# thenoobychocobo/gpt2-image-captioning

Measured on AMD Instinct MI355X. Metric: training images/sec + greedy captions/sec, GPT2-small+CLIP-B/32 at 1/2/4/8 GPU, higher is better.
Workload: dtype bf16

## Files before the change

### gpt2-image-captioning_amd/csrc/elementwise.hip

```cpp
#include "common.h"

#include <math.h>

namespace icap {

static inline hipStream_t S_(void* s) { return reinterpret_cast<hipStream_t>(s); }
static inline unsigned nblk(int64_t n, int per, int cap = 65535) {
  int64_t b = (n + per - 1) / per;
  if (b < 1) b = 1;
  if (b > cap) b = cap;
  return (unsigned)b;
}

__device__ __forceinline__ float block_sum256(float v, float* red) {
  v = wave_sum(v);
  const int lane = threadIdx.x & 63, w = threadIdx.x >> 6;
  __syncthreads();
  if (lane == 0) red[w] = v;
  __syncthreads();
  float r = red[0] + red[1] + red[2] + red[3];
  return r;
}

template <typename T>
__global__ void gpt2_embed_kernel(int B, int P, int L, int D, const T* __restrict__ prefix, int64_t pbs,
                                  const T* __restrict__ wte, const T* __restrict__ wpe,
                                  const int64_t* __restrict__ ids, T* __restrict__ x, uint32_t thr,
                                  float inv_keep, uint64_t seed0, const uint64_t* seed_ptr, uint64_t offset,
                                  const int32_t* __restrict__ seq_off, const int32_t* __restrict__ seq_len) {
  const int S = P + L, D4 = D >> 2;
  const uint64_t seed = thr ? eff_seed(seed0, seed_ptr) : 0ull;
  const int64_t total = (int64_t)B * S * D4;
  for (int64_t i = (int64_t)blockIdx.x * blockDim.x + threadIdx.x; i < total; i += (int64_t)gridDim.x * blockDim.x) {
    const int64_t prow = i / D4;
    const int c = (int)(i - prow * D4) * 4;
    const int b = (int)(prow / S), t = (int)(prow - (int64_t)b * S);
    int64_t row = prow;
    if (seq_off) {
      if (t >= seq_len[b]) continue;
      row = (int64_t)seq_off[b] + t;
    }
    float v[4], w[4];
    if (t < P) io<T>::ld4(prefix + (int64_t)b * pbs + (int64_t)t * D + c, v);
    else io<T>::ld4(wte + ids[(int64_t)b * L + (t - P)] * D + c, v);
    io<T>::ld4(wpe + (int64_t)t * D + c, w);
#pragma unroll
    for (int e = 0; e < 4; ++e) {
      v[e] += w[e];
      if (thr) v[e] *= drop_scale(seed, offset + (uint64_t)(row * D + c + e), thr, inv_keep);
    }
    io<T>::st4(x + row * D + c, v);
  }
}

template <typename T>
// ... 495 lines not shown
  const double lr = (double)lr0 * lam;
  const double t = (double)(k + 1);
  const double bc1 = 1.0 - pow((double)beta1, t);
  const double bc2 = 1.0 - pow((double)beta2, t);
  st->norm = norm;
  st->clip = clip;
  st->lr = (float)lr;
  st->step_size = (float)(lr / bc1);
  st->bc2_sqrt = (float)sqrt(bc2);
  st->decay = (float)(1.0 - lr * (double)wd);
  st->step = k + 1;
}

__device__ __forceinline__ void adam_one(float& p, float g, float& m, float& v, float clip, float decay, float w1,
                                         float b2, float w2, float step_size, float bc2s, float eps) {
  g *= clip;
  p *= decay;
  m = m + w1 * (g - m);
  v = v * b2 + w2 * (g * g);
  const float denom = sqrtf(v) / bc2s + eps;
  p = p + (-step_size) * (m / denom);
}

__global__ __launch_bounds__(256) void adam_update_kernel(int64_t n, float* __restrict__ P, const float* __restrict__ G,
                                                         float* __restrict__ M1, float* __restrict__ M2,
                                                         bf16_t* __restrict__ out16, const AdamState* __restrict__ st,
                                                         float beta1, float beta2, float eps) {
  const float clip = st->clip, decay = st->decay, step_size = st->step_size, bc2s = st->bc2_sqrt;
  const float w1 = 1.f - beta1, w2 = 1.f - beta2;
  const int64_t n4 = n >> 2;
  for (int64_t i = (int64_t)blockIdx.x * 256 + threadIdx.x; i < n4; i += (int64_t)gridDim.x * 256) {
    float4 p = reinterpret_cast<float4*>(P)[i];
    const float4 g = reinterpret_cast<const float4*>(G)[i];
    float4 m = reinterpret_cast<float4*>(M1)[i];
    float4 v = reinterpret_cast<float4*>(M2)[i];
    adam_one(p.x, g.x, m.x, v.x, clip, decay, w1, beta2, w2, step_size, bc2s, eps);
    adam_one(p.y, g.y, m.y, v.y, clip, decay, w1, beta2, w2, step_size, bc2s, eps);
    adam_one(p.z, g.z, m.z, v.z, clip, decay, w1, beta2, w2, step_size, bc2s, eps);
    adam_one(p.w, g.w, m.w, v.w, clip, decay, w1, beta2, w2, step_size, bc2s, eps);
    reinterpret_cast<float4*>(P)[i] = p;
    reinterpret_cast<float4*>(M1)[i] = m;
    reinterpret_cast<float4*>(M2)[i] = v;
    if (out16) {
      const float o[4] = {p.x, p.y, p.z, p.w};
      io<bf16_t>::st4(out16 + 4 * i, o);
    }
  }
  if (blockIdx.x == 0) {
    for (int64_t i = 4 * n4 + threadIdx.x; i < n; i += 256) {
      float p = P[i], m = M1[i], v = M2[i];
      adam_one(p, G[i], m, v, clip, decay, w1, beta2, w2, step_size, bc2s, eps);
      P[i] = p; M1[i] = m; M2[i] = v;
      if (out16) out16[i] = f2bf(p);
    }
  }
}

template <typename T>
__global__ __launch_bounds__(256) void transpose_kernel(int64_t rows, int64_t cols, const T* __restrict__ src,
                                                       int64_t lds, T* __restrict__ dst, int64_t ldd,
                                                       int64_t rows_pad) {
  __shared__ T tile[64][65];
  const int64_t r0 = (int64_t)blockIdx.y * 64, c0 = (int64_t)blockIdx.x * 64;
  const int tx = threadIdx.x & 63, ty = threadIdx.x >> 6;
  for (int i = ty; i < 64; i += 4) {
    const int64_t r = r0 + i, c = c0 + tx;
    T v = (T)0;
    if (r < rows && c < cols) v = src[r * lds + c];
    tile[i][tx] = v;
  }
  __syncthreads();
  for (int i = ty; i < 64; i += 4) {
    const int64_t c = c0 + i, r = r0 + tx;
    if (c < cols && r < rows_pad) dst[c * ldd + r] = tile[tx][i];
  }
}

template <typename T>
__global__ __launch_bounds__(256) void colsum_kernel(int64_t M, int64_t N, const T* __restrict__ src, int64_t ld,
                                                    int64_t rows_per_chunk, float* __restrict__ partial) {
  __shared__ float red[4][64];
  const int tx = threadIdx.x & 63, ty = threadIdx.x >> 6;
  const int64_t c = (int64_t)blockIdx.x * 64 + tx;
  const int64_t m0 = (int64_t)blockIdx.y * rows_per_chunk;
  int64_t m1 = m0 + rows_per_chunk;
  if (m1 > M) m1 = M;
  float a = 0.f;
  if (c < N)
    for (int64_t m = m0 + ty; m < m1; m += 4) a += io<T>::ld(src + m * ld + c);
  red[ty][tx] = a;
  __syncthreads();
  if (ty == 0 && c < N) partial[(int64_t)blockIdx.y * N + c] = red[0][tx] + red[1][tx] + red[2][tx] + red[3][tx];
}

constexpr int T16_TLD = 68;
__device__ __forceinline__ void transpose16_tile(int64_t rows, int64_t cols, const uint16_t* __restrict__ src,
                                                 int64_t lds, uint16_t* __restrict__ dst, int64_t ldd, int64_t r0,
                                                 int64_t c0, uint16_t* tile) {
  constexpr int TLD = T16_TLD;
#pragma unroll
  for (int h = 0; h < 2; ++h) {
    const int idx = threadIdx.x + 256 * h;
    const int r = idx >> 3, ch = idx & 7;
    uint4 v = make_uint4(0, 0, 0, 0);
    if (r0 + r < rows && c0 + 8 * ch < cols) v = *reinterpret_cast<const uint4*>(src + (r0 + r) * lds + c0 + 8 * ch);
    uint2* t = reinterpret_cast<uint2*>(&tile[r * TLD + 8 * ch]);
// ... 745 lines not shown
  ICAP_REQUIRE(V > 0 && ld >= V && ld % 4 == 0, "icap_cross_entropy: ld must be >= V and a multiple of 4");
  if (rows <= 0) return ICAP_OK;
  ICAP_REQUIRE(rows < (1ll << 31), "icap_cross_entropy: too many rows");
  float* lrows = reinterpret_cast<float*>(workspace);
  const bool reg = dtype == ICAP_BF16 && V <= 8 * 512 * 13 && ld % 8 == 0 &&
                   (reinterpret_cast<uintptr_t>(logits) & 15) == 0 &&
                   (dlogits == nullptr || (reinterpret_cast<uintptr_t>(dlogits) & 15) == 0);
  if (reg) {
    hipLaunchKernelGGL(ce_bf16_reg_kernel<13>, dim3((unsigned)rows), dim3(512), 0, S_(stream), V,
                       reinterpret_cast<const bf16_t*>(logits), ld, labels, n_valid, lrows,
                       reinterpret_cast<bf16_t*>(dlogits), grad_scale, rows_dev);
  } else {
    DISPATCH_T(dtype, hipLaunchKernelGGL(ce_kernel<T>, dim3((unsigned)rows), dim3(256), 0, S_(stream), V, CTP(logits),
                                         ld, labels, n_valid, lrows, TP(dlogits), grad_scale, rows_dev));
  }
  int rc = check_launch("icap_cross_entropy");
  if (rc) return rc;
  hipLaunchKernelGGL(ce_reduce_kernel, dim3(1), dim3(256), 0, S_(stream), rows, lrows, n_valid, loss, rows_dev);
  return check_launch("icap_cross_entropy(reduce)");
}

extern "C" size_t icap_adamw_workspace_bytes(int64_t n) {
  (void)n;
  return SQ_BLOCKS * sizeof(float);
}

static int sq_partials(int64_t n, const float* x, float* partial, hipStream_t s, int* nparts) {
  const int nb = (int)nblk(n / 4 + 1, 256, SQ_BLOCKS);
  hipLaunchKernelGGL(sqnorm_partial_kernel, dim3(nb), dim3(256), 0, s, n, x, partial);
  *nparts = nb;
  return check_launch("sqnorm");
}

extern "C" int icap_sqnorm(int64_t n, const float* x, float* out, void* workspace, void* stream) {
  ICAP_REQUIRE(x && out && workspace, "icap_sqnorm: null pointer");
  ICAP_REQUIRE((reinterpret_cast<uintptr_t>(x) & 15) == 0, "icap_sqnorm: x must be 16-byte aligned");
  int np = 0;
  float* partial = reinterpret_cast<float*>(workspace);
  int rc = sq_partials(n, x, partial, S_(stream), &np);
  if (rc) return rc;
  hipLaunchKernelGGL(adam_finalize_kernel, dim3(1), dim3(256), 0, S_(stream), np, partial, (AdamState*)nullptr, out,
                     0.f, 0.f, 0.f, 0.f, 0.f, (int64_t)0, (int64_t)0);
  return check_launch("icap_sqnorm");
}

extern "C" int icap_adamw_step(const icap_adamw_args* a, void* workspace, void* stream) {
  ICAP_REQUIRE(a && workspace, "icap_adamw_step: null args/workspace");
  ICAP_REQUIRE(a->params && a->grads && a->exp_avg && a->exp_avg_sq && a->state, "icap_adamw_step: null pointer");
  ICAP_REQUIRE(((reinterpret_cast<uintptr_t>(a->params) | reinterpret_cast<uintptr_t>(a->grads) |
                 reinterpret_cast<uintptr_t>(a->exp_avg) | reinterpret_cast<uintptr_t>(a->exp_avg_sq)) & 15) == 0,
               "icap_adamw_step: buffers must be 16-byte aligned");
  ICAP_REQUIRE(a->bf16_out == nullptr || (reinterpret_cast<uintptr_t>(a->bf16_out) & 7) == 0,
               "icap_adamw_step: bf16_out must be 8-byte aligned");
  if (a->n <= 0) return ICAP_OK;
  hipStream_t s = S_(stream);
  float* partial = reinterpret_cast<float*>(workspace);
  int np = 0;
  int rc = sq_partials(a->n, a->grads, partial, s, &np);
  if (rc) return rc;
  hipLaunchKernelGGL(adam_finalize_kernel, dim3(1), dim3(256), 0, s, np, partial, (AdamState*)a->state,
                     (float*)nullptr, a->lr, a->beta1, a->beta2, a->weight_decay, a->max_norm, a->num_warmup_steps,
                     a->num_training_steps);
  rc = check_launch("icap_adamw_step(finalize)");
  if (rc) return rc;
  hipLaunchKernelGGL(adam_update_kernel, dim3(nblk(a->n / 4 + 1, 256, 4096)), dim3(256), 0, s, a->n, a->params,
                     a->grads, a->exp_avg, a->exp_avg_sq, (bf16_t*)a->bf16_out, (const AdamState*)a->state, a->beta1,
                     a->beta2, a->eps);
  return check_launch("icap_adamw_step(update)");
}

extern "C" int icap_transpose(int32_t dtype, int64_t rows, int64_t cols, const void* src, int64_t lds, void* dst,
                              int64_t ldd, int64_t rows_pad, void* stream) {
  ICAP_REQUIRE(src && dst && rows_pad >= rows, "icap_transpose: bad args");
  if (rows_pad == 0 || cols == 0) return ICAP_OK;
  dim3 grid((unsigned)((cols + 63) / 64), (unsigned)((rows_pad + 63) / 64));
  ICAP_REQUIRE(grid.y < 65536, "icap_transpose: too many rows");
  const bool vec = dtype == ICAP_BF16 && cols % 8 == 0 && lds % 8 == 0 && ldd % 8 == 0 && rows_pad % 64 == 0 &&
                   (reinterpret_cast<uintptr_t>(src) & 15) == 0 && (reinterpret_cast<uintptr_t>(dst) & 15) == 0;
  if (vec)
    hipLaunchKernelGGL(transpose16_vec_kernel, grid, dim3(256), 0, S_(stream), rows, cols, (const uint16_t*)src, lds,
                       (uint16_t*)dst, ldd);
  else if (dtype == ICAP_BF16)
    hipLaunchKernelGGL(transpose_kernel<uint16_t>, grid, dim3(256), 0, S_(stream), rows, cols, (const uint16_t*)src,
                       lds, (uint16_t*)dst, ldd, rows_pad);
  else
    hipLaunchKernelGGL(transpose_kernel<uint32_t>, grid, dim3(256), 0, S_(stream), rows, cols, (const uint32_t*)src,
                       lds, (uint32_t*)dst, ldd, rows_pad);
  return check_launch("icap_transpose");
}

extern "C" int icap_transpose_batch(int32_t n, const icap_transpose_item* items, void* stream) {
  ICAP_REQUIRE(n >= 0 && (n == 0 || items), "icap_transpose_batch: bad args");
  for (int32_t i0 = 0; i0 < n; i0 += T16_BATCH) {
    const int m = n - i0 < T16_BATCH ? n - i0 : T16_BATCH;
    Transpose16Batch b;
    b.n = 0;
    b.off[0] = 0;
    for (int j = 0; j < m; ++j) {
      const icap_transpose_item& it = items[i0 + j];
      ICAP_REQUIRE(it.src && it.dst && it.rows >= 0 && it.cols >= 0, "icap_transpose_batch: bad item");
      if (it.rows == 0 || it.cols == 0) continue;
      const bool vec = it.cols % 8 == 0 && it.lds % 8 == 0 && it.ldd % 8 == 0 && it.rows % 64 == 0 &&
                       it.lds >= it.cols && it.ldd >= it.rows && (reinterpret_cast<uintptr_t>(it.src) & 15) == 0 &&
                       (reinterpret_cast<uintptr_t>(it.dst) & 15) == 0;
      if (!vec) {
        const int rc = icap_transpose(ICAP_BF16, it.rows, it.cols, it.src, it.lds, it.dst, it.ldd, it.rows, stream);
        if (rc) return rc;
        continue;
      }
      const int k = b.n++;
      b.src[k] = static_cast<const uint16_t*>(it.src);
      b.dst[k] = static_cast<uint16_t*>(it.dst);
      b.rows[k] = it.rows; b.cols[k] = it.cols; b.lds[k] = it.lds; b.ldd[k] = it.ldd;
      b.off[k + 1] = b.off[k] + ((it.cols + 63) / 64) * (it.rows / 64);
    }
    if (b.n == 0) continue;
    ICAP_REQUIRE(b.off[b.n] < (1ll << 31), "icap_transpose_batch: too many tiles");
    hipLaunchKernelGGL(transpose16_batch_kernel, dim3((unsigned)b.off[b.n]), dim3(256), 0, S_(stream), b);
    const int rc = check_launch("icap_transpose_batch");
    if (rc) return rc;
  }
// ... 288 lines not shown
```

### gpt2-image-captioning_amd/icap/_lib.py

```python

from __future__ import annotations

import ctypes as C
import os

import torch

_HERE = os.path.dirname(os.path.abspath(__file__))
LIB_PATH = os.environ.get("ICAP_LIB") or os.path.join(_HERE, "libicap_hip.so")

F32, BF16, FP8_MX = 0, 1, 2
ACT_NONE, ACT_GELU_NEW, ACT_RELU, ACT_QUICK_GELU, ACT_TANH, ACT_GELU_ERF = 0, 1, 2, 3, 4, 5
AGG_MEAN, AGG_MAX, AGG_SUM_NORM = 0, 1, 2

vp = C.c_void_p
i32, i64, u64, f32, sz = C.c_int32, C.c_int64, C.c_uint64, C.c_float, C.c_size_t
pi32 = C.POINTER(C.c_int32)
pi64 = C.POINTER(C.c_int64)


class GemmArgs(C.Structure):
    _fields_ = [
        ("M", i64), ("N", i64), ("K", i64),
        ("in_dtype", i32), ("c_dtype", i32),
# ... 14 lines not shown
        ("trans_ab", i32),
        ("ln_gamma", vp), ("ln_beta", vp), ("ln_eps", f32),
        ("path", i32),
        ("a_scale", vp), ("b_scale", vp),
        ("m_hint", i64),
        ("tickets", vp), ("tickets_len", i64),
        ("ln_wsum", vp),
        ("ln_stats_out", vp), ("ln_stats_in", vp), ("ln_mean_out", vp), ("ln_rstd_out", vp),
        ("diag_stamps", vp),
    ]


class LnParamItem(C.Structure):
    _fields_ = [("workspace", vp), ("rows", i64), ("D", i64), ("dgamma", vp), ("dbeta", vp), ("overwrite", i32)]


class TransposeItem(C.Structure):
    _fields_ = [("src", vp), ("lds", i64), ("dst", vp), ("ldd", i64), ("rows", i64), ("cols", i64)]


class ColsumItem(C.Structure):
    _fields_ = [("src", vp), ("ld", i64), ("N", i64), ("out", vp)]


class AttnArgs(C.Structure):
    _fields_ = [
        ("dtype", i32),
        ("B", i32), ("S", i32), ("H", i32), ("hd", i32),
        ("row_stride_b", i64), ("row_stride_s", i64),
        ("qkv", vp), ("ld_qkv", i64),
        ("out", vp), ("ld_out", i64),
        ("lse", vp),
        ("key_mask", vp),
        ("causal", i32),
        ("scale", f32),
        ("drop_p", f32), ("seed", u64), ("offset", u64),
        ("seed_ptr", vp),
        ("dout", vp), ("ld_dout", i64),
        ("dqkv", vp), ("ld_dqkv", i64),
        ("seq_off", vp), ("seq_len", vp),
        ("short_only", i32),
    ]


class AdamWArgs(C.Structure):
    _fields_ = [
        ("n", i64),
        ("params", vp), ("grads", vp), ("exp_avg", vp), ("exp_avg_sq", vp),
        ("bf16_out", vp),
        ("state", vp),
        ("lr", f32), ("beta1", f32), ("beta2", f32), ("eps", f32), ("weight_decay", f32),
        ("max_norm", f32),
        ("num_warmup_steps", i64), ("num_training_steps", i64),
    ]


class BeamArgs(C.Structure):
    _fields_ = [
        ("B", i32), ("W", i32), ("V", i32), ("max_len", i32),
        ("eos", i32), ("length_penalty", f32),
        ("K", i32),
        ("T", i32),
        ("top_val", vp), ("top_idx", vp), ("top_m", vp), ("top_ls", vp),
        ("ws", vp),
        ("dtype", i32), ("D", i32), ("n_positions", i32),
        ("wte", vp), ("wpe", vp), ("x", vp),
    ]


SIGNATURES = {
    "icap_last_error": (C.c_char_p, []),
    "icap_version": (C.c_int, []),
    "icap_device_arch_ok": (C.c_int, []),
    "icap_gemm": (C.c_int, [C.POINTER(GemmArgs), vp]),
    "icap_gemm_group": (C.c_int, [C.POINTER(GemmArgs), C.c_int32, vp]),
    "icap_gemm_kernel_name": (C.c_char_p, [C.POINTER(GemmArgs)]),
    "icap_gemm_plan_info": (C.c_int, [C.POINTER(GemmArgs), vp, vp]),
    "icap_mx_scale_bytes": (sz, [i64, i64]),
    "icap_quantize_mx": (C.c_int, [i32, i64, i64, vp, i64, vp, i64, vp, vp, vp]),
    "icap_layernorm_fwd": (C.c_int, [i32, i64, i64, vp, i64, vp, vp, f32, vp, i64, vp, vp, vp, vp, vp]),
    "icap_layernorm_bwd_workspace_bytes": (sz, [i64, i64]),
    "icap_layernorm_bwd": (C.c_int, [i32, i64, i64, vp, i64, vp, vp, vp, vp, i64, vp, i64, vp, i64, vp,
                                     f32, u64, u64, vp, vp, vp, vp, vp, vp, i32, vp]),
    "icap_ln_param_reduce_batch": (C.c_int, [i32, C.POINTER(LnParamItem), vp]),
    "icap_attention_fwd": (C.c_int, [C.POINTER(AttnArgs), vp]),
    "icap_attention_bwd": (C.c_int, [C.POINTER(AttnArgs), vp]),
    "icap_attention_decode": (C.c_int, [i32, i32, i32, i32, i32, vp, i64, vp, i64, f32, vp]),
    "icap_attention_decode_anc": (C.c_int, [i32, i32, i32, i32, i32, vp, i64, vp, vp, i64, f32, vp]),
    "icap_beam_workspace_bytes": (C.c_size_t, [i32, i32, i32, i32]),
    "icap_beam_layout": (C.c_int, [i32, i32, i32, i32, vp]),
    "icap_beam_init": (C.c_int, [C.POINTER(BeamArgs), i32, vp]),
    "icap_beam_rowtop": (C.c_int, [i32, i64, i64, vp, i64, i32, vp, vp, vp, vp, vp]),
    "icap_beam_update": (C.c_int, [C.POINTER(BeamArgs), i32, i32, vp]),
    "icap_beam_finalize": (C.c_int, [C.POINTER(BeamArgs), vp, vp, vp]),
    "icap_gpt2_embed": (C.c_int, [i32, i32, i32, i32, i32, vp, i64, vp, vp, vp, vp, f32, u64, u64, vp, vp, vp, vp]),
    "icap_embedding_scatter_add": (C.c_int, [i32, i32, i32, i32, i32, vp, vp, vp, vp]),
    "icap_caption_prep": (C.c_int, [i32, i32, i32, vp, vp, vp, vp, vp, vp, vp, vp]),
    "icap_caption_pack": (C.c_int, [i32, i32, i32, vp, vp, vp, vp, vp, vp, vp, vp, vp, vp, vp]),
    "icap_rows_unpack": (C.c_int, [i32, i32, i32, i32, vp, vp, vp, vp, i64, vp]),
    "icap_cross_entropy_workspace_bytes": (sz, [i64]),
    "icap_cross_entropy": (C.c_int, [i32, i64, i64, vp, i64, vp, vp, vp, vp, f32, vp, vp, vp]),
    "icap_adamw_workspace_bytes": (sz, [i64]),
    "icap_adamw_step": (C.c_int, [C.POINTER(AdamWArgs), vp, vp]),
    "icap_sqnorm": (C.c_int, [i64, vp, vp, vp, vp]),
    "icap_transpose": (C.c_int, [i32, i64, i64, vp, i64, vp, i64, i64, vp]),
    "icap_transpose_batch": (C.c_int, [i32, vp, vp]),
    "icap_colsum_workspace_bytes": (sz, [i64, i64]),
# ... 76 lines not shown
```

### gpt2-image-captioning_amd/icap/engine.py

```python

from __future__ import annotations

from types import SimpleNamespace
from typing import List, Optional, Tuple

import torch

from . import ops
from .mapper import DWHelper, MLPMapperCore, TransformerMapperCore
from .models import _embedding_grads

SHORT_ONLY = True
GRAD_OVERWRITE = True

Tensor = torch.Tensor


def _async_src(t: Tensor) -> bool:
    return t.device.type != "cpu" or t.is_pinned()


class CaptionTrainer:
    def __init__(self, model, batch_size: int, caption_len: int, *, lr: float = 1e-4, weight_decay: float = 0.01,
                 betas=(0.9, 0.999), eps: float = 1e-8, max_norm: float = 1.0, num_warmup_steps: int = 0,
                 num_training_steps: int = 1, dropout: bool = True, seed: int = 0, clip_model=None,
                 grad_accum_steps: int = 1, process_group=None, compact_head: bool = True,
                 pack_rows: bool = True, dp_overlap: bool = True, dp_bf16: bool = False, force_overlap: bool = False,
                 mapper_dw: str = "fused"):
        self.model = model
        self.dtype = model.compute_dtype
        self.B, self.Lc = batch_size, caption_len
        self.hp = SimpleNamespace(lr=lr, weight_decay=weight_decay, betas=betas, eps=eps, max_norm=max_norm,
                                  num_warmup_steps=num_warmup_steps, num_training_steps=num_training_steps)
        self.dropout = dropout
        self.seed = seed
        self.grad_accum_steps = grad_accum_steps
        self.pg = process_group
        self.world = 1
        self.distributed = process_group is not None or (torch.distributed.is_available()
                                                         and torch.distributed.is_initialized())
        if self.distributed:
            self.world = torch.distributed.get_world_size(process_group)
            broadcast_replicas([model] + ([clip_model] if clip_model is not None else []), process_group)
        self.force_overlap = bool(force_overlap) and self.distributed
        self.dev = model.device
        flat = model.flat()
        self.flat = flat
        self.mcore = model.mapping_network.core(self.dtype, flat)
        self.clip = clip_model.core(self.dtype) if clip_model is not None else None
        self.gpt_trainable = not model.freeze_gpt_weights
        if self.gpt_trainable:
            model.gpt.invalidate_core()
            self.gcore = model.gpt.core(self.dtype)
            model.gpt.invalidate_core()
            self.gcore.bind_flat(flat)
            compact_head = False
        else:
            self.gcore = model.gpt.core(self.dtype)
        B, Lc = batch_size, caption_len
        P = model.total_prefix_length
        self.P = P
        per_layer = (dict(per_layer_grads=mapper_dw in ("side", "group")) if isinstance(self.mcore, TransformerMapperCore)
                     else {})
        self.mws = self.mcore.alloc(B, train=True, **per_layer)
        self.gws = self.gcore.alloc_train(B, P, Lc, keep_for_dw=self.gpt_trainable, compact_head=compact_head,
                                          pack=pack_rows)
# ... 118 lines not shown
                d_pre = st.d_emb.view(B, S * D)[:, : P * D]
                mc.backward_from(d_pre[:, : Pm * D], S * D, self.mws, self.emb_c, self.mgrads, self.dwh)

            segs.append((self._ranges_mapper[0], mlp))
        last_rng, last_fn = segs[-1]

        def last():
            last_fn()
            self.loss_sum.add_(self.gws.loss)

        segs[-1] = (last_rng, last)
        return segs

    def _overwrite_ok(self) -> bool:
        return GRAD_OVERWRITE and isinstance(self.mcore, TransformerMapperCore) and not self.gpt_trainable

    def _front(self, zero: bool, grad_scale: float):
        B, P, D = self.B, self.P, self.gcore.D
        model = self.model
        if zero and not self._overwrite_ok():
            self.flat.flat_grad.zero_()
        if self.clip is not None:
            emb = self.clip.run(self.cws, self.pixels)
            ops.convert(emb, self.emb_c)
        else:
            ops.convert(self.emb, self.emb_c)
        if self.dropout:
            ops.counter_increment(self.counter)
        mc, gc = self.mcore, self.gcore
        mc.forward(self.mws, self.emb_c, self.mdr, train=True)
        pre, pbs = mc.prefix_view(self.mws)
        if model.task_prefix_embeds is not None:
            Pm = mc.P
            ops.convert(_rows_view(pre, B, Pm * D, pbs), self.pre.view(B, P * D)[:, : Pm * D])
            ops.broadcast_rows(model.task_prefix_embeds.data, self.pre.view(-1)[Pm * D:], B, P * D)
            pre, pbs = self.pre, P * D
        gc.forward_train(self.gws, pre, pbs, self.ids, self.mask, self.labels, self.gdr, fuse_dlogits=True,
                         grad_scale=grad_scale)
        S = self.gws.S
        d_emb = gc.backward(self.gws, self.gdr, self.gws.key_mask, self.gws.logits, grads=self.ggrads,
                            dw=self.dwh if self.gpt_trainable else None)
        if self.gpt_trainable:
            _embedding_grads(d_emb, self.ids, B, P, self.Lc, D, self.ggrads, self.dwh)
        d_pre = d_emb.view(B, S * D)[:, : P * D]
        Pm = mc.P
        if model.task_prefix_embeds is not None:
            ops.colsum(d_emb.view(B, S * D)[:, Pm * D: P * D], self.task_grad.view(-1), self.dwh.cs_ws,
                       accumulate=not (zero and self._overwrite_ok()), M=B, N=(P - Pm) * D)
        if isinstance(mc, TransformerMapperCore):
            Hl, Sm = mc.Hl, mc.S
            ops.convert(d_pre[:, : Pm * D], self.mws.dout.view(B, Sm * D)[:, Hl * D:])
        return d_emb

    def _optimizer(self) -> None:
        hp, f = self.hp, self.flat
        ops.adamw_step(f.flat, f.flat_grad, f.exp_avg, f.exp_avg_sq, self.adam_state, self.adam_ws, lr=hp.lr,
                       betas=hp.betas, eps=hp.eps, weight_decay=hp.weight_decay, max_norm=hp.max_norm,
                       num_warmup_steps=hp.num_warmup_steps, num_training_steps=hp.num_training_steps,
                       bf16_out=f.flat_c)
        self.mcore.refresh_transposes()
        if self.gpt_trainable:
            self.gcore.refresh_from_flat()

    def _allreduce(self) -> None:
        if self.world > 1:
            if self.dp_bf16:
                g = self.flat.flat_grad
                self._to16(g, 0, g.numel())
                torch.distributed.all_reduce(self._g16, group=self.pg)
                self._from16(g, [(0, g.numel())])
            else:
                torch.distributed.all_reduce(self.flat.flat_grad, group=self.pg)

    def _to16(self, g, lo: int, hi: int) -> None:
        if self._g16 is None:
            self._g16 = torch.empty(g.numel(), dtype=torch.bfloat16, device=g.device)
        if g.is_cuda:
            ops.convert(g[lo:hi].view(1, -1), self._g16[lo:hi].view(1, -1))
        else:
            self._g16[lo:hi].copy_(g[lo:hi])

    def _from16(self, g, ranges) -> None:
        for lo, hi in ranges:
            if g.is_cuda:
                ops.convert(self._g16[lo:hi].view(1, -1), g[lo:hi].view(1, -1))
            else:
                g[lo:hi].copy_(self._g16[lo:hi])

    def _bucket(self, ranges, works) -> None:
        g = self.flat.flat_grad
        if not ranges:
            return
        src = (lambda lo, hi: self._g16[lo:hi]) if self.dp_bf16 else (lambda lo, hi: g[lo:hi])
        if g.is_cuda:
            if self._comm is None:
                self._comm = torch.cuda.Stream(g.device)
            ev = torch.cuda.Event()
            ev.record()
            with torch.cuda.stream(self._comm):
                self._comm.wait_event(ev)
                for lo, hi in ranges:
                    if self.dp_bf16:
                        self._to16(g, lo, hi)
                    works.append(torch.distributed.all_reduce(src(lo, hi), group=self.pg, async_op=True))
        else:
            for lo, hi in ranges:
                if self.dp_bf16:
                    self._to16(g, lo, hi)
                works.append(torch.distributed.all_reduce(src(lo, hi), group=self.pg, async_op=True))
        if self.dp_bf16:
            self._pending16.extend(ranges)

    def _overlapped_step(self, zero: bool, use_graph: bool) -> None:
# ... 171 lines not shown
```

### gpt2-image-captioning_amd/icap/mapper.py

```python

from __future__ import annotations

import math
from types import SimpleNamespace
from typing import Optional

import torch
import torch.nn as nn

from . import _lib as L
from . import ops
from .ops import Dropout
from .weights import det_tensor

Tensor = torch.Tensor


def _rup(x: int, m: int) -> int:
    return (x + m - 1) // m * m




def _kout_ok(t: Tensor) -> bool:
# ... 207 lines not shown


def _compute_view(flat, p: nn.Parameter, dtype: torch.dtype) -> Tensor:
    if flat is not None:
        return flat.view_c(p)
    if dtype == torch.float32:
        return p.data
    t = torch.empty(p.shape, dtype=dtype, device=p.device)
    ops.convert(p.data.reshape(p.shape[0], -1), t.reshape(p.shape[0], -1))
    return t


class TransformerMapperCore:

    def __init__(self, m: TransformerMappingNetwork, dtype: torch.dtype, flat=None):
        from ._lib import require_device

        self.m, self.dtype, self.flat = m, dtype, flat
        self.dev = m.linear.weight.device
        require_device(self.dev)
        self.D, self.E = m.gpt_dim, m.embed_dim
        self.H = m.nhead
        self.hd = self.D // self.H
        self.Hl, self.P = m.hidden_length, m.prefix_length
        self.S = self.Hl + self.P
        self.nl = len(m.transformer.layers)
        self.refresh()

    @torch.no_grad()
    def refresh(self) -> None:
        m, dt = self.m, self.dtype
        cv = lambda p: _compute_view(self.flat, p, dt)
        self.w_lin, self.b_lin = cv(m.linear.weight), m.linear.bias.data
        self.prefix_const = m.prefix_const.data
        self.layers = []
        for lay in m.transformer.layers:
            w = SimpleNamespace()
            w.in_w, w.in_b = cv(lay.self_attn.in_proj_weight), lay.self_attn.in_proj_bias.data
            w.out_w, w.out_b = cv(lay.self_attn.out_proj.weight), lay.self_attn.out_proj.bias.data
            w.l1_w, w.l1_b = cv(lay.linear1.weight), lay.linear1.bias.data
            w.l2_w, w.l2_b = cv(lay.linear2.weight), lay.linear2.bias.data
            w.n1_g, w.n1_b = lay.norm1.weight.data, lay.norm1.bias.data
            w.n2_g, w.n2_b = lay.norm2.weight.data, lay.norm2.bias.data
            w.in_wt = torch.empty((w.in_w.shape[1], w.in_w.shape[0]), dtype=dt, device=self.dev)
            w.out_wt = torch.empty((w.out_w.shape[1], w.out_w.shape[0]), dtype=dt, device=self.dev)
            w.l1_wt = torch.empty((w.l1_w.shape[1], w.l1_w.shape[0]), dtype=dt, device=self.dev)
            w.l2_wt = torch.empty((w.l2_w.shape[1], w.l2_w.shape[0]), dtype=dt, device=self.dev)
            self.layers.append(w)
        self.refresh_transposes()

    def dw_cols(self) -> int:
        return max(self.Hl * self.D, 4 * self.D, self.E)

    def refresh_transposes(self) -> None:
        pairs = [(a, b) for w in self.layers
                 for a, b in ((w.in_w, w.in_wt), (w.out_w, w.out_wt), (w.l1_w, w.l1_wt), (w.l2_w, w.l2_wt))]
        if pairs and pairs[0][0].dtype == torch.bfloat16:
            ops.transpose_batch(pairs)
        else:
            for a, b in pairs:
                ops.transpose(a, b)

    def grads(self, flat) -> SimpleNamespace:
        m = self.m
        g = SimpleNamespace(lin_w=flat.grad(m.linear.weight), lin_b=flat.grad(m.linear.bias),
                            prefix_const=flat.grad(m.prefix_const), layers=[])
        for lay in m.transformer.layers:
            g.layers.append(SimpleNamespace(
                in_w=flat.grad(lay.self_attn.in_proj_weight), in_b=flat.grad(lay.self_attn.in_proj_bias),
                out_w=flat.grad(lay.self_attn.out_proj.weight), out_b=flat.grad(lay.self_attn.out_proj.bias),
                l1_w=flat.grad(lay.linear1.weight), l1_b=flat.grad(lay.linear1.bias),
                l2_w=flat.grad(lay.linear2.weight), l2_b=flat.grad(lay.linear2.bias),
                n1_g=flat.grad(lay.norm1.weight), n1_b=flat.grad(lay.norm1.bias),
                n2_g=flat.grad(lay.norm2.weight), n2_b=flat.grad(lay.norm2.bias)))
        return g

    def alloc(self, B: int, train: bool, per_layer_grads: bool = False) -> SimpleNamespace:
        S, D, dt, dev, nl = self.S, self.D, self.dtype, self.dev, self.nl
        M = B * S
        e = lambda *shape, dtype=dt: torch.empty(shape, dtype=dtype, device=dev)
        ws = SimpleNamespace(B=B, M=M, S=S)
        n_keep = nl if train else 1
        ws.x = [e(M, D) for _ in range(nl + 1)] if train else [e(M, D), e(M, D)]
        ws.a1 = [e(M, D) for _ in range(n_keep)]
        ws.qkv = [e(M, 3 * D) for _ in range(n_keep)]
        ws.o = [e(M, D) for _ in range(n_keep)]
        ws.h1 = [e(M, D) for _ in range(n_keep)]
        ws.a2 = [e(M, D) for _ in range(n_keep)]
        ws.f = [e(M, 4 * D) for _ in range(n_keep)]
        ws.mean1 = [e(M, dtype=torch.float32) for _ in range(n_keep)]
        ws.rstd1 = [e(M, dtype=torch.float32) for _ in range(n_keep)]
        ws.mean2 = [e(M, dtype=torch.float32) for _ in range(n_keep)]
        ws.rstd2 = [e(M, dtype=torch.float32) for _ in range(n_keep)]
        ws.lse = [e(B * self.H * S, dtype=torch.float32) for _ in range(n_keep)]
        if train:
            ws.dout = torch.zeros((M, D), dtype=dt, device=dev)
            ws.dres = e(M, D)
            n_set = nl if per_layer_grads else 1
            n_alt = nl if per_layer_grads else min(2, nl)

            def bufs(n, cols):
                b = [e(M, cols) for _ in range(n)]
                return [b[l % n] for l in range(nl)]

            ws.g_r = bufs(n_alt, D)
            ws.g_rm = bufs(n_set, D)
            ws.g_m = bufs(n_alt, D)
            ws.g_mm = bufs(n_set, D)
            ws.g_dz = bufs(n_set, 4 * D)
# ... 237 lines not shown
```

### gpt2-image-captioning_amd/icap/ops.py

```python

from __future__ import annotations

import contextlib
import ctypes as C
import os
import gc
from typing import Optional, Tuple

import torch

from . import _lib as L
from ._lib import AdamWArgs, AttnArgs, GemmArgs, call

Tensor = torch.Tensor


def dtype_code(t: torch.dtype) -> int:
    if t == torch.float32:
        return L.F32
    if t == torch.bfloat16:
        return L.BF16
    raise L.IcapError(f"unsupported storage dtype {t} (float32 or bfloat16)")


# ... 517 lines not shown
                 key_mask: Optional[Tensor], labels_shift: Optional[Tensor], n_valid: Optional[Tensor],
                 row_slot: Optional[Tensor] = None, labels_compact: Optional[Tensor] = None) -> None:
    for t in (mask, labels):
        if t is not None and t.dtype != torch.int64:
            raise L.IcapError("caption_prep: mask/labels must be int64")
    call("icap_caption_prep", B, P, L_, _p(mask), _p(labels), _p(key_mask), _p(labels_shift), _p(n_valid),
         _p(row_slot), _p(labels_compact), _stream())


def caption_pack(B: int, P: int, L_: int, mask: Optional[Tensor], labels: Tensor, seq_off: Tensor, seq_len: Tensor,
                 m_live: Tensor, key_mask: Tensor, labels_shift: Tensor, n_valid: Optional[Tensor],
                 row_slot: Optional[Tensor] = None, labels_compact: Optional[Tensor] = None) -> None:
    for t in (mask, labels):
        if t is not None and t.dtype != torch.int64:
            raise L.IcapError("caption_pack: mask/labels must be int64")
    for t in (seq_off, seq_len, m_live, key_mask, labels_shift):
        if t.dtype != torch.int32:
            raise L.IcapError("caption_pack: outputs must be int32")
    call("icap_caption_pack", B, P, L_, _p(mask), _p(labels), seq_off.data_ptr(), seq_len.data_ptr(),
         m_live.data_ptr(), key_mask.data_ptr(), labels_shift.data_ptr(), _p(n_valid), _p(row_slot),
         _p(labels_compact), _stream())


def rows_unpack(src: Tensor, seq_off: Tensor, seq_len: Tensor, dst: Tensor, *, B: int, P: int, D: int,
                dst_bstride: int) -> Tensor:
    if src.dtype != dst.dtype:
        raise L.IcapError("rows_unpack: src and dst must share a dtype")
    call("icap_rows_unpack", dtype_code(src.dtype), B, P, D, src.data_ptr(), seq_off.data_ptr(), seq_len.data_ptr(),
         dst.data_ptr(), dst_bstride, _stream())
    return dst


def cross_entropy_workspace(rows: int) -> int:
    return int(L.load().icap_cross_entropy_workspace_bytes(rows))


def cross_entropy(logits: Tensor, V: int, labels: Tensor, n_valid: Tensor, loss: Tensor,
                  dlogits: Optional[Tensor], workspace: Tensor, grad_scale: float = 1.0,
                  rows: Optional[int] = None, rows_dev: Optional[Tensor] = None) -> Tensor:
    rows = logits.shape[0] if rows is None else rows
    call("icap_cross_entropy", dtype_code(logits.dtype), rows, V, logits.data_ptr(), _ld(logits),
         labels.data_ptr(), n_valid.data_ptr(), loss.data_ptr(), _p(dlogits), grad_scale, workspace.data_ptr(),
         _p(rows_dev), _stream())
    return loss


def adamw_workspace(n: int) -> int:
    return int(L.load().icap_adamw_workspace_bytes(n))


def adamw_step(params: Tensor, grads: Tensor, exp_avg: Tensor, exp_avg_sq: Tensor, state: Tensor,
               workspace: Tensor, *, lr: float, betas=(0.9, 0.999), eps: float = 1e-8,
               weight_decay: float = 0.01, max_norm: float = 1.0, num_warmup_steps: int = 0,
               num_training_steps: int = 1, bf16_out: Optional[Tensor] = None) -> None:
    a = AdamWArgs()
    a.n = params.numel()
    a.params, a.grads, a.exp_avg, a.exp_avg_sq = (params.data_ptr(), grads.data_ptr(), exp_avg.data_ptr(),
                                                  exp_avg_sq.data_ptr())
    a.bf16_out = _p(bf16_out)
    a.state = state.data_ptr()
    a.lr, a.beta1, a.beta2, a.eps, a.weight_decay = lr, betas[0], betas[1], eps, weight_decay
    a.max_norm = max_norm
    a.num_warmup_steps, a.num_training_steps = num_warmup_steps, num_training_steps
    call("icap_adamw_step", C.byref(a), workspace.data_ptr(), _stream())


def sqnorm(x: Tensor, out: Tensor, workspace: Tensor) -> Tensor:
    call("icap_sqnorm", x.numel(), x.data_ptr(), out.data_ptr(), workspace.data_ptr(), _stream())
    return out


def transpose(src: Tensor, dst: Tensor, rows_pad: Optional[int] = None, rows: Optional[int] = None,
              cols: Optional[int] = None) -> Tensor:
    rows = src.shape[0] if rows is None else rows
    cols = src.shape[1] if cols is None else cols
    call("icap_transpose", dtype_code(src.dtype), rows, cols, src.data_ptr(), _ld(src), dst.data_ptr(), _ld(dst),
         rows if rows_pad is None else rows_pad, _stream())
    return dst


def transpose_batch(pairs) -> None:
    pairs = list(pairs)
    if not pairs:
        return
    items = (L.TransposeItem * len(pairs))()
    for it, (src, dst) in zip(items, pairs):
        if src.dtype != torch.bfloat16 or dst.dtype != torch.bfloat16:
            raise L.IcapError("transpose_batch: bf16 matrices only")
        it.src, it.lds, it.dst, it.ldd = src.data_ptr(), _ld(src), dst.data_ptr(), _ld(dst)
        it.rows, it.cols = src.shape[0], src.shape[1]
    call("icap_transpose_batch", len(pairs), C.cast(items, C.c_void_p), _stream())


def colsum_workspace(M: int, N: int) -> int:
    return int(L.load().icap_colsum_workspace_bytes(M, N))


def colsum(src: Tensor, out: Tensor, workspace: Tensor, accumulate: bool = True, M: Optional[int] = None,
           N: Optional[int] = None) -> Tensor:
    M = src.shape[0] if M is None else M
    N = src.shape[1] if N is None else N
    call("icap_colsum", dtype_code(src.dtype), M, N, src.data_ptr(), _ld(src), out.data_ptr(),
         1 if accumulate else 0, workspace.data_ptr(), _stream())
    return out


COLSUM_BATCH = 16

# ... 219 lines not shown
```

### include/icap.h

```cpp
#ifndef ICAP_H
#define ICAP_H

#include <stddef.h>
#include <stdint.h>

#ifdef __cplusplus
extern "C" {
#endif

enum { ICAP_F32 = 0, ICAP_BF16 = 1, ICAP_FP8_MX = 2 };
enum {
  ICAP_ACT_NONE = 0,
  ICAP_ACT_GELU_NEW = 1,
  ICAP_ACT_RELU = 2,
  ICAP_ACT_QUICK_GELU = 3,
  ICAP_ACT_TANH = 4,
  ICAP_ACT_GELU_ERF = 5
};
enum { ICAP_OK = 0, ICAP_ERR_ARG = 1, ICAP_ERR_LAUNCH = 2 };

const char* icap_last_error(void);
int icap_version(void);
int icap_device_arch_ok(void);

// ... 52 lines not shown
int icap_ln_param_reduce_batch(int32_t n, const icap_ln_param_item* items, void* stream);

typedef struct {
  int32_t dtype;
  int32_t B, S, H, hd;
  int64_t row_stride_b, row_stride_s;
  const void* qkv; int64_t ld_qkv;
  void* out; int64_t ld_out;
  float* lse;
  const int32_t* key_mask;
  int32_t causal;
  float scale;
  float drop_p; uint64_t seed; uint64_t offset;
  const uint64_t* seed_ptr;
  const void* dout; int64_t ld_dout;
  void* dqkv; int64_t ld_dqkv;
  const int32_t* seq_off; const int32_t* seq_len;
  int32_t short_only;
} icap_attn_args;
int icap_attention_fwd(const icap_attn_args* a, void* stream);
int icap_attention_bwd(const icap_attn_args* a, void* stream);

int icap_attention_decode(int32_t dtype, int32_t B, int32_t H, int32_t hd, int32_t pos,
                          const void* cache, int64_t ld_cache, void* out, int64_t ld_out,
                          float scale, void* stream);
int icap_attention_decode_anc(int32_t dtype, int32_t B, int32_t H, int32_t hd, int32_t pos,
                              const void* cache, int64_t ld_cache, const int32_t* anc, void* out,
                              int64_t ld_out, float scale, void* stream);

int icap_gpt2_embed(int32_t dtype, int32_t B, int32_t P, int32_t L, int32_t D,
                    const void* prefix, int64_t prefix_bstride, const void* wte,
                    const void* wpe, const int64_t* ids, void* x, float drop_p,
                    uint64_t seed, uint64_t offset, const uint64_t* seed_ptr,
                    const int32_t* seq_off, const int32_t* seq_len, void* stream);
int icap_embedding_scatter_add(int32_t dtype, int32_t B, int32_t P, int32_t L, int32_t D,
                               const void* dx, const int64_t* ids, float* dwte, void* stream);
int icap_caption_prep(int32_t B, int32_t P, int32_t L, const int64_t* mask,
                      const int64_t* labels, int32_t* key_mask, int32_t* labels_shift,
                      int32_t* n_valid, int32_t* row_slot, int32_t* labels_compact, void* stream);
int icap_caption_pack(int32_t B, int32_t P, int32_t L, const int64_t* mask, const int64_t* labels,
                      int32_t* seq_off, int32_t* seq_len, int32_t* m_live, int32_t* key_mask,
                      int32_t* labels_shift, int32_t* n_valid, int32_t* row_slot, int32_t* labels_compact,
                      void* stream);
int icap_rows_unpack(int32_t dtype, int32_t B, int32_t P, int32_t D, const void* src, const int32_t* seq_off,
                     const int32_t* seq_len, void* dst, int64_t dst_bstride, void* stream);

size_t icap_cross_entropy_workspace_bytes(int64_t rows);
int icap_cross_entropy(int32_t dtype, int64_t rows, int64_t V, const void* logits, int64_t ld,
                       const int32_t* labels, const int32_t* n_valid, float* loss,
                       void* dlogits, float grad_scale, void* workspace, const int32_t* rows_dev,
                       void* stream);

typedef struct {
  int64_t n;
  float* params; float* grads; float* exp_avg; float* exp_avg_sq;
  void* bf16_out;
  void* state;
  float lr, beta1, beta2, eps, weight_decay;
  float max_norm;
  int64_t num_warmup_steps, num_training_steps;
} icap_adamw_args;
size_t icap_adamw_workspace_bytes(int64_t n);
int icap_adamw_step(const icap_adamw_args* a, void* workspace, void* stream);
int icap_sqnorm(int64_t n, const float* x, float* out, void* workspace, void* stream);

int icap_transpose(int32_t dtype, int64_t rows, int64_t cols, const void* src, int64_t lds,
                   void* dst, int64_t ldd, int64_t rows_pad, void* stream);
typedef struct {
  const void* src; int64_t lds; void* dst; int64_t ldd; int64_t rows; int64_t cols;
} icap_transpose_item;
int icap_transpose_batch(int32_t n, const icap_transpose_item* items, void* stream);
size_t icap_colsum_workspace_bytes(int64_t M, int64_t N);
int icap_colsum(int32_t dtype, int64_t M, int64_t N, const void* src, int64_t ld, float* out,
                int32_t accumulate, void* workspace, void* stream);
#define ICAP_COLSUM_BATCH 16
typedef struct {
  const void* src; int64_t ld; int64_t N; float* out;
} icap_colsum_item;
int icap_colsum_batch(int32_t dtype, int64_t M, int32_t n, const icap_colsum_item* items, int32_t accumulate,
                      void* workspace, void* stream);
int icap_dropout_apply(int32_t dtype, int64_t M, int64_t N, const void* src, int64_t lds,
                       void* dst, int64_t ldd, float drop_p, uint64_t seed, uint64_t offset,
                       const uint64_t* seed_ptr, void* stream);
int icap_counter_increment(uint64_t* counter, void* stream);
int icap_convert(int32_t src_dtype, int32_t dst_dtype, int64_t M, int64_t N, const void* src,
                 int64_t lds, void* dst, int64_t ldd, void* stream);
int icap_broadcast_rows(int32_t dtype, int32_t B, int64_t R, int64_t D, const float* src,
                        void* dst, int64_t dst_bstride, void* stream);

int icap_im2col_patches(int32_t dtype, int32_t B, int32_t C, int32_t HW, int32_t patch,
                        const float* pixels, void* patches, void* stream);
int icap_vit_embed(int32_t dtype, int32_t B, int32_t G2, int32_t D, const void* patch_emb,
                   const float* cls, const float* pos, void* x, void* stream);
int icap_patch_embed(int32_t B, int32_t C, int32_t HW, int32_t patch, int32_t NP, int32_t N, const float* pixels,
                     const void* w, int64_t ldw, int32_t Kp, const float* bias, const float* pos, const float* prefix,
                     void* out, int64_t ldo, void* stream);
int icap_prefix_embed(int32_t dtype, int32_t B, int32_t G2, int32_t NP, int32_t D, const void* patch_emb,
                      const float* prefix, const float* pos, void* x, void* stream);
int icap_rope_patches(int32_t dtype, int32_t B, int32_t S, int32_t NP, int32_t H, int32_t hd, void* qkv,
                      int64_t ld_qkv, const float* cos_t, const float* sin_t, void* stream);
int icap_l2norm_rows(int32_t dtype, int64_t rows, int64_t D, const void* x, int64_t ldx,
                     float* out, int64_t ldo, void* stream);

int icap_greedy_next(int32_t dtype, int32_t B, int64_t V, const void* logits, int64_t ld,
                     int64_t eos, const int64_t* forced, int32_t* finished, int64_t* tokens, int64_t ld_tokens,
                     int32_t step, const void* wte, const void* wpe, int32_t pos, int32_t D,
                     void* x, void* stream);
int icap_topp_sample(int32_t dtype, int32_t B, int64_t V, const void* logits, int64_t ld, float temperature,
                     float top_p, const int32_t* finished, uint64_t seed, const uint64_t* seed_ptr,
                     int32_t step, int64_t eos, int64_t* out, void* stream);
typedef struct {
  int32_t B, W, V, max_len;
  int32_t eos; float length_penalty;
// ... 39 lines not shown
```

Baseline: 14600.

## Fuse mapper weight transposes into the AdamW update kernel

Adds a segmented AdamW kernel that, for mapper weight matrices inside the flat buffer, writes the bf16 copy and also stages it through shared memory to write the transposed copy. This removes the separate transpose_batch pass after the optimizer step. It also switches the param and moment loads and stores to nontemporal accesses. The cost is a host-side plan (sort, std::vector, a large struct passed by value as a kernel argument), a linear segment search in every block, and a fallback transpose for items that cannot be tiled.

```diff
diff --git a/gpt2-image-captioning_amd/csrc/elementwise.hip b/gpt2-image-captioning_amd/csrc/elementwise.hip
--- a/gpt2-image-captioning_amd/csrc/elementwise.hip
+++ b/gpt2-image-captioning_amd/csrc/elementwise.hip
@@ -1,6 +1,9 @@
 #include "common.h"
 
 #include <math.h>
+
+#include <algorithm>
+#include <vector>
 
 namespace icap {
 
@@ -602,6 +605,117 @@
       adam_one(p, G[i], m, v, clip, decay, w1, beta2, w2, step_size, bc2s, eps);
       P[i] = p; M1[i] = m; M2[i] = v;
       if (out16) out16[i] = f2bf(p);
+    }
+  }
+}
+
+constexpr int ADAM_ITEMS = 32;
+constexpr int ADAM_SEGS = 2 * ADAM_ITEMS + 1;
+constexpr int ADAM_TR = 64, ADAM_TC = 256, ADAM_TLD = ADAM_TC + 2;
+constexpr int ADAM_UNIT4 = 4096;
+struct AdamPlan {
+  int nseg;
+  int32_t off[ADAM_SEGS + 1];
+  int64_t start[ADAM_SEGS];
+  int64_t rows[ADAM_SEGS];
+  int64_t cols[ADAM_SEGS];
+  uint16_t* dst[ADAM_SEGS];
+  int64_t ldd[ADAM_SEGS];
+};
+
+typedef float adam_f4_t __attribute__((ext_vector_type(4)));
+__device__ __forceinline__ float4 adam_ld4(const float* x, int64_t i4) {
+  const adam_f4_t t = __builtin_nontemporal_load(reinterpret_cast<const adam_f4_t*>(x) + i4);
+  return make_float4(t.x, t.y, t.z, t.w);
+}
+__device__ __forceinline__ void adam_st4(float* x, int64_t i4, const float4& v) {
+  const adam_f4_t t = {v.x, v.y, v.z, v.w};
+  __builtin_nontemporal_store(t, reinterpret_cast<adam_f4_t*>(x) + i4);
+}
+
+__global__ __launch_bounds__(256) void adam_update_items_kernel(int64_t n, float* __restrict__ P,
+                                                               const float* __restrict__ G, float* __restrict__ M1,
+                                                               float* __restrict__ M2, bf16_t* __restrict__ out16,
+                                                               const AdamState* __restrict__ st, float beta1,
+                                                               float beta2, float eps, AdamPlan pl) {
+  __shared__ __attribute__((aligned(16))) uint16_t tile[ADAM_TR * ADAM_TLD];
+  const float clip = st->clip, decay = st->decay, step_size = st->step_size, bc2s = st->bc2_sqrt;
+  const float w1 = 1.f - beta1, w2 = 1.f - beta2;
+  const int bid = blockIdx.x, tid = threadIdx.x;
+  int s = 0;
+  while (s + 1 < pl.nseg && bid >= pl.off[s + 1]) ++s;
+  const int64_t u = bid - pl.off[s];
+  const int64_t base = pl.start[s], rows = pl.rows[s], cols = pl.cols[s];
+  int64_t r0 = 0, c0 = 0;
+  const int lane = tid & 63, w = tid >> 6;
+  if (rows) {
+    const int64_t tx = (cols + ADAM_TC - 1) / ADAM_TC;
+    const int64_t ty = u / tx;
+    r0 = ty * ADAM_TR;
+    c0 = (u - ty * tx) * ADAM_TC;
+  }
+#pragma unroll 1
+  for (int k0 = 0; k0 < 16; k0 += 4) {
+    int64_t i4[4];
+    float4 p[4], g[4], m[4], v[4];
+#pragma unroll
+    for (int q = 0; q < 4; ++q) {
+      const int k = k0 + q;
+      if (rows) {
+        const int64_t c = c0 + 4 * lane;
+        i4[q] = c < cols ? (base + (r0 + w + 4 * k) * cols + c) >> 2 : -1;
+      } else {
+        const int64_t j = u * ADAM_UNIT4 + k * 256 + tid;
+        i4[q] = j < cols ? (base >> 2) + j : -1;
+      }
+      if (i4[q] >= 0) {
+        p[q] = adam_ld4(P, i4[q]);
+        g[q] = reinterpret_cast<const float4*>(G)[i4[q]];
+        m[q] = adam_ld4(M1, i4[q]);
+        v[q] = adam_ld4(M2, i4[q]);
+      }
+    }
+#pragma unroll
+    for (int q = 0; q < 4; ++q) {
+      if (i4[q] < 0) continue;
+      adam_one(p[q].x, g[q].x, m[q].x, v[q].x, clip, decay, w1, beta2, w2, step_size, bc2s, eps);
+      adam_one(p[q].y, g[q].y, m[q].y, v[q].y, clip, decay, w1, beta2, w2, step_size, bc2s, eps);
+      adam_one(p[q].z, g[q].z, m[q].z, v[q].z, clip, decay, w1, beta2, w2, step_size, bc2s, eps);
+      adam_one(p[q].w, g[q].w, m[q].w, v[q].w, clip, decay, w1, beta2, w2, step_size, bc2s, eps);
+      adam_st4(P, i4[q], p[q]);
+      adam_st4(M1, i4[q], m[q]);
+      adam_st4(M2, i4[q], v[q]);
+      const uint2 o = make_uint2(f2bf2(p[q].x, p[q].y), f2bf2(p[q].z, p[q].w));
+      *reinterpret_cast<uint2*>(out16 + 4 * i4[q]) = o;
+      if (rows) {
+        uint32_t* t = reinterpret_cast<uint32_t*>(&tile[(w + 4 * (k0 + q)) * ADAM_TLD + 4 * lane]);
+        t[0] = o.x;
+        t[1] = o.y;
+      }
+    }
+  }
+  if (rows) {
+    __syncthreads();
+    uint16_t* dst = pl.dst[s];
+    const int64_t ldd = pl.ldd[s];
+#pragma unroll
+    for (int h = 0; h < 8; ++h) {
+      const int idx = tid + 256 * h;
+      const int rq = idx & 7, c = idx >> 3;
+      if (c0 + c >= cols) continue;
+      uint32_t x[4];
+#pragma unroll
+      for (int e = 0; e < 4; ++e)
+        x[e] = (uint32_t)tile[(8 * rq + 2 * e) * ADAM_TLD + c] | ((uint32_t)tile[(8 * rq + 2 * e + 1) * ADAM_TLD + c] << 16);
+      *reinterpret_cast<uint4*>(dst + (c0 + c) * ldd + r0 + 8 * rq) = make_uint4(x[0], x[1], x[2], x[3]);
+    }
+  }
+  if (bid == 0) {
+    for (int64_t i = (n & ~(int64_t)3) + tid; i < n; i += 256) {
+      float p = P[i], m = M1[i], v = M2[i];
+      adam_one(p, G[i], m, v, clip, decay, w1, beta2, w2, step_size, bc2s, eps);
+      P[i] = p; M1[i] = m; M2[i] = v;
+      out16[i] = f2bf(p);
     }
   }
 }
@@ -1453,6 +1567,60 @@
                "icap_adamw_step: buffers must be 16-byte aligned");
   ICAP_REQUIRE(a->bf16_out == nullptr || (reinterpret_cast<uintptr_t>(a->bf16_out) & 7) == 0,
                "icap_adamw_step: bf16_out must be 8-byte aligned");
+  AdamPlan pl;
+  pl.nseg = 0;
+  pl.off[0] = 0;
+  std::vector<icap_transpose_item> rest_v;
+  ICAP_REQUIRE(a->n_items >= 0 && (a->n_items == 0 || (a->items && a->bf16_out)),
+               "icap_adamw_step: items need an item array and bf16_out");
+  if (a->n_items > 0) {
+    std::vector<icap_adamw_item> its(a->items, a->items + a->n_items);
+    std::sort(its.begin(), its.end(),
+              [](const icap_adamw_item& x, const icap_adamw_item& y) { return x.offset < y.offset; });
+    const bool out_ok = (reinterpret_cast<uintptr_t>(a->bf16_out) & 15) == 0;
+    int64_t cur = 0, total = 0;
+    int taken = 0;
+    auto flat_run = [&](int64_t lo, int64_t hi) {
+      const int64_t len4 = (hi - lo) >> 2;
+      if (len4 <= 0) return;
+      const int k = pl.nseg++;
+      pl.start[k] = lo; pl.rows[k] = 0; pl.cols[k] = len4; pl.dst[k] = nullptr; pl.ldd[k] = 0;
+      total += (len4 + ADAM_UNIT4 - 1) / ADAM_UNIT4;
+      pl.off[k + 1] = (int32_t)total;
+    };
+    int64_t prev_end = 0;
+    for (const icap_adamw_item& it : its) {
+      ICAP_REQUIRE(it.dst && it.offset >= 0 && it.rows >= 0 && it.cols >= 0 && it.ldd >= it.rows &&
+                       (it.cols == 0 || it.rows <= (a->n - it.offset) / it.cols) && it.offset <= a->n,
+                   "icap_adamw_step: item outside the flat buffer or ldd < rows");
+      ICAP_REQUIRE(it.offset >= prev_end, "icap_adamw_step: items overlap");
+      const int64_t end = it.offset + it.rows * it.cols;
+      prev_end = end;
+      if (it.rows == 0 || it.cols == 0) continue;
+      const bool tile = out_ok && taken < ADAM_ITEMS && it.offset % 8 == 0 && it.rows % ADAM_TR == 0 &&
+                        it.cols % 8 == 0 && it.ldd % 8 == 0 && (reinterpret_cast<uintptr_t>(it.dst) & 15) == 0;
+      if (!tile) {
+        rest_v.push_back(icap_transpose_item{static_cast<const uint16_t*>(a->bf16_out) + it.offset, it.cols, it.dst,
+                                             it.ldd, it.rows, it.cols});
+        continue;
+      }
+      flat_run(cur, it.offset);
+      const int k = pl.nseg++;
+      pl.start[k] = it.offset; pl.rows[k] = it.rows; pl.cols[k] = it.cols;
+      pl.dst[k] = static_cast<uint16_t*>(it.dst); pl.ldd[k] = it.ldd;
+      total += (it.rows / ADAM_TR) * ((it.cols + ADAM_TC - 1) / ADAM_TC);
+      ICAP_REQUIRE(total < (1ll << 31), "icap_adamw_step: too many tiles");
+      pl.off[k + 1] = (int32_t)total;
+      cur = end;
+      ++taken;
+    }
+    if (taken) {
+      flat_run(cur, a->n);
+      ICAP_REQUIRE(total < (1ll << 31), "icap_adamw_step: too many blocks");
+    }
+  }
+  const int32_t n_rest = (int32_t)rest_v.size();
+  const icap_transpose_item* rest = rest_v.data();
   if (a->n <= 0) return ICAP_OK;
   hipStream_t s = S_(stream);
   float* partial = reinterpret_cast<float*>(workspace);
@@ -1464,10 +1632,19 @@
                      a->num_training_steps);
   rc = check_launch("icap_adamw_step(finalize)");
   if (rc) return rc;
-  hipLaunchKernelGGL(adam_update_kernel, dim3(nblk(a->n / 4 + 1, 256, 4096)), dim3(256), 0, s, a->n, a->params,
-                     a->grads, a->exp_avg, a->exp_avg_sq, (bf16_t*)a->bf16_out, (const AdamState*)a->state, a->beta1,
-                     a->beta2, a->eps);
-  return check_launch("icap_adamw_step(update)");
+  if (pl.nseg == 0) {
+    hipLaunchKernelGGL(adam_update_kernel, dim3(nblk(a->n / 4 + 1, 256, 4096)), dim3(256), 0, s, a->n, a->params,
+                       a->grads, a->exp_avg, a->exp_avg_sq, (bf16_t*)a->bf16_out, (const AdamState*)a->state,
+                       a->beta1, a->beta2, a->eps);
+    rc = check_launch("icap_adamw_step(update)");
+  } else {
+    hipLaunchKernelGGL(adam_update_items_kernel, dim3((unsigned)pl.off[pl.nseg]), dim3(256), 0, s, a->n, a->params,
+                       a->grads, a->exp_avg, a->exp_avg_sq, (bf16_t*)a->bf16_out, (const AdamState*)a->state,
+                       a->beta1, a->beta2, a->eps, pl);
+    rc = check_launch("icap_adamw_step(update + transposed copies)");
+  }
+  if (rc || n_rest == 0) return rc;
+  return icap_transpose_batch(n_rest, rest, stream);
 }
 
 extern "C" int icap_transpose(int32_t dtype, int64_t rows, int64_t cols, const void* src, int64_t lds, void* dst,
diff --git a/gpt2-image-captioning_amd/icap/_lib.py b/gpt2-image-captioning_amd/icap/_lib.py
--- a/gpt2-image-captioning_amd/icap/_lib.py
+++ b/gpt2-image-captioning_amd/icap/_lib.py
@@ -90,7 +90,12 @@
         ("lr", f32), ("beta1", f32), ("beta2", f32), ("eps", f32), ("weight_decay", f32),
         ("max_norm", f32),
         ("num_warmup_steps", i64), ("num_training_steps", i64),
-    ]
+        ("n_items", i32), ("items", vp),
+    ]
+
+
+class AdamWItem(C.Structure):
+    _fields_ = [("offset", i64), ("rows", i64), ("cols", i64), ("dst", vp), ("ldd", i64)]
 
 
 class BeamArgs(C.Structure):
diff --git a/gpt2-image-captioning_amd/icap/engine.py b/gpt2-image-captioning_amd/icap/engine.py
--- a/gpt2-image-captioning_amd/icap/engine.py
+++ b/gpt2-image-captioning_amd/icap/engine.py
@@ -12,6 +12,7 @@
 
 SHORT_ONLY = True
 GRAD_OVERWRITE = True
+ADAM_TRANSPOSE = True
 
 Tensor = torch.Tensor
 
@@ -236,13 +237,27 @@
             ops.convert(d_pre[:, : Pm * D], self.mws.dout.view(B, Sm * D)[:, Hl * D:])
         return d_emb
 
+    def _adam_items(self):
+        f = self.flat
+        if f.flat_c is None or f.flat_c.dtype != torch.bfloat16 or not isinstance(self.mcore, TransformerMapperCore):
+            return None
+        base, end = f.flat_c.data_ptr(), f.flat_c.data_ptr() + 2 * f.n
+        items = []
+        for a, b in self.mcore.transpose_pairs():
+            if not (base <= a.data_ptr() < end and a.is_contiguous()):
+                return None
+            items.append(((a.data_ptr() - base) // 2, a.shape[0], a.shape[1], b))
+        return items
+
     def _optimizer(self) -> None:
         hp, f = self.hp, self.flat
+        items = self._adam_items() if ADAM_TRANSPOSE else None
         ops.adamw_step(f.flat, f.flat_grad, f.exp_avg, f.exp_avg_sq, self.adam_state, self.adam_ws, lr=hp.lr,
                        betas=hp.betas, eps=hp.eps, weight_decay=hp.weight_decay, max_norm=hp.max_norm,
                        num_warmup_steps=hp.num_warmup_steps, num_training_steps=hp.num_training_steps,
-                       bf16_out=f.flat_c)
-        self.mcore.refresh_transposes()
+                       bf16_out=f.flat_c, items=items)
+        if not items:
+            self.mcore.refresh_transposes()
         if self.gpt_trainable:
             self.gcore.refresh_from_flat()
 
diff --git a/gpt2-image-captioning_amd/icap/mapper.py b/gpt2-image-captioning_amd/icap/mapper.py
--- a/gpt2-image-captioning_amd/icap/mapper.py
+++ b/gpt2-image-captioning_amd/icap/mapper.py
@@ -283,9 +283,12 @@
     def dw_cols(self) -> int:
         return max(self.Hl * self.D, 4 * self.D, self.E)
 
+    def transpose_pairs(self):
+        return [(a, b) for w in self.layers
+                for a, b in ((w.in_w, w.in_wt), (w.out_w, w.out_wt), (w.l1_w, w.l1_wt), (w.l2_w, w.l2_wt))]
+
     def refresh_transposes(self) -> None:
-        pairs = [(a, b) for w in self.layers
-                 for a, b in ((w.in_w, w.in_wt), (w.out_w, w.out_wt), (w.l1_w, w.l1_wt), (w.l2_w, w.l2_wt))]
+        pairs = self.transpose_pairs()
         if pairs and pairs[0][0].dtype == torch.bfloat16:
             ops.transpose_batch(pairs)
         else:
diff --git a/gpt2-image-captioning_amd/icap/ops.py b/gpt2-image-captioning_amd/icap/ops.py
--- a/gpt2-image-captioning_amd/icap/ops.py
+++ b/gpt2-image-captioning_amd/icap/ops.py
@@ -593,8 +593,18 @@
 def adamw_step(params: Tensor, grads: Tensor, exp_avg: Tensor, exp_avg_sq: Tensor, state: Tensor,
                workspace: Tensor, *, lr: float, betas=(0.9, 0.999), eps: float = 1e-8,
                weight_decay: float = 0.01, max_norm: float = 1.0, num_warmup_steps: int = 0,
-               num_training_steps: int = 1, bf16_out: Optional[Tensor] = None) -> None:
+               num_training_steps: int = 1, bf16_out: Optional[Tensor] = None, items=None) -> None:
     a = AdamWArgs()
+    arr = None
+    if items:
+        if bf16_out is None:
+            raise L.IcapError("adamw_step: items need bf16_out")
+        arr = (L.AdamWItem * len(items))()
+        for it, (off, rows, cols, dst) in zip(arr, items):
+            if dst.dtype != torch.bfloat16 or dst.dim() != 2 or tuple(dst.shape) != (cols, rows):
+                raise L.IcapError("adamw_step: an item's dst must be a bf16 [cols, rows] matrix")
+            it.offset, it.rows, it.cols, it.dst, it.ldd = off, rows, cols, dst.data_ptr(), _ld(dst)
+        a.n_items, a.items = len(items), C.cast(arr, C.c_void_p)
     a.n = params.numel()
     a.params, a.grads, a.exp_avg, a.exp_avg_sq = (params.data_ptr(), grads.data_ptr(), exp_avg.data_ptr(),
                                                   exp_avg_sq.data_ptr())
diff --git a/include/icap.h b/include/icap.h
--- a/include/icap.h
+++ b/include/icap.h
@@ -128,6 +128,9 @@
                        void* stream);
 
 typedef struct {
+  int64_t offset; int64_t rows; int64_t cols; void* dst; int64_t ldd;
+} icap_adamw_item;
+typedef struct {
   int64_t n;
   float* params; float* grads; float* exp_avg; float* exp_avg_sq;
   void* bf16_out;
@@ -135,6 +138,8 @@
   float lr, beta1, beta2, eps, weight_decay;
   float max_norm;
   int64_t num_warmup_steps, num_training_steps;
+  int32_t n_items;
+  const icap_adamw_item* items;
 } icap_adamw_args;
 size_t icap_adamw_workspace_bytes(int64_t n);
 int icap_adamw_step(const icap_adamw_args* a, void* workspace, void* stream);
```

After: 14750 (median of 6 runs). 1.0% higher.
